# lab4d-org/lab4d

Measured on AMD Instinct MI355X. Metric: rendered rays/sec (fwd+bwd) at 512² × 128 samples; PSNR vs ref, higher is better.
Workload: dtype bf16

## Files before the change

### include/lab4d_hip.h

```cpp
#ifndef LAB4D_HIP_H
#define LAB4D_HIP_H

#include <stdint.h>

#ifdef __cplusplus
extern "C" {
#endif

#define LAB4D_OK 0
#define LAB4D_EINVAL (-1)
#define LAB4D_ELAUNCH (-2)

#define LAB4D_F32 0
#define LAB4D_F16 1
#define LAB4D_F64 2

const char* lab4d_last_error(void);
int lab4d_version(void);
const char* lab4d_arch(void);
const char* lab4d_build_flags(void);

int lab4d_quaternion_mul_forward(const void* in1, const void* in2, void* out, uint32_t B, uint32_t D1,
                                 uint32_t D2, int dtype, void* stream);
int lab4d_quaternion_mul_backward(const void* grad, uint32_t B, uint32_t D1, uint32_t D2, const void* in1,
// ... 22 lines not shown

int lab4d_sample_pdf(const float* bins, const float* weights, int R, int n_w, int n_imp, float eps,
                     float* samples, int64_t* inds, void* stream);
int lab4d_sample_pdf_u(const float* bins, const float* weights, const float* u_sorted, int R, int n_w, int n_imp, float eps,
                       float* samples, int64_t* inds, void* stream);
int lab4d_sort_depth(const float* a, int na, const float* b, int nb, int R, float* out, void* stream);

int lab4d_valid_mask(const float* xyz, const float* xyz_t, const float* aabb, const float* t_aabb, long S, unsigned char* mask, void* stream);
long lab4d_compact_work_ints(long S);
int lab4d_compact(const unsigned char* mask, long S, int* idx, int* count, int* work, void* stream);
int lab4d_gather_rows(const float* src, const int* idx, const int* count, long n_rows, int C, float* dst, void* stream);
int lab4d_scatter_rows(const float* src, const int* idx, const int* count, long n_rows, int C, float* dst, void* stream);
int lab4d_frame_of(const int* idx, const int* count, long n_rows, int spf, int* frame, void* stream);

#define LAB4D_MAX_FIELDS 16
typedef struct {
  int n_fields;
  const float* fields[LAB4D_MAX_FIELDS];
  int channels[LAB4D_MAX_FIELDS];
  int modes[LAB4D_MAX_FIELDS];
} lab4d_field_list;
typedef struct {
  int n_fields;
  float* fields[LAB4D_MAX_FIELDS];
} lab4d_field_grads;

int lab4d_composite_forward(const float* density, const float* deltas, const lab4d_field_list* fl,
                            const float* flow, const float* vis, const float* gauss_density, int R, int D,
                            float* weights, float* transmit, float* mask, float* out, float* flow_out,
                            float* vis_num, float* t_sum, float* gauss_mask, void* stream);
// ... 61 lines not shown
```

### lab4d_amd/_lib.py

```python
import ctypes
import os
import re
import subprocess
import sys
from concurrent.futures import ThreadPoolExecutor

import torch

HERE = os.path.dirname(os.path.abspath(__file__))
ROOT = os.path.dirname(HERE)
CSRC = os.path.join(HERE, "csrc")
INCLUDE = os.path.join(ROOT, "include")
SO_PATH = os.environ.get("LAB4D_SO_PATH", os.path.join(HERE, "liblab4d_hip.so"))
BUILD_DIR = os.environ.get("LAB4D_BUILD_DIR", os.path.join(HERE, "build"))
HIPCC = os.environ.get("HIPCC", "/opt/rocm/bin/hipcc")
ARCH = "gfx950"
CFLAGS = ["--offload-arch=" + ARCH, "-O3", "-std=c++17", "-fPIC", "-I" + INCLUDE, "-I" + CSRC,
          "-Wno-unused-value", "-Wno-pass-failed"] + os.environ.get("LAB4D_HIPCC_EXTRA", "").split()


MLP_INST_FLAGS = ["-mllvm", "-amdgpu-disable-unclustered-high-rp-reschedule"]


def sources():
# ... 114 lines not shown
    def bind(cls):
        MIRRORS[c_name] = cls
        if _LIB is not None:
            for name, (_, params, _) in SIGNATURES.items():
                if c_name in params:
                    getattr(_LIB, name).argtypes = argtypes(params)
        return cls
    return bind


@mirrors("lab4d_field_list")
class FieldList(ctypes.Structure):
    _fields_ = [("n_fields", ci), ("fields", vp * 16), ("channels", ci * 16), ("modes", ci * 16)]


@mirrors("lab4d_field_grads")
class FieldGrads(ctypes.Structure):
    _fields_ = [("n_fields", ci), ("fields", vp * 16)]


def lib():
    global _LIB
    if _LIB is None:
        if not os.path.exists(SO_PATH):
            raise RuntimeError(
                "liblab4d_hip.so is missing (%s). Build it with `python -c 'import __graft_entry__ as g; g.build()'`; "
                "lab4d_amd has no CPU or eager-PyTorch fallback." % SO_PATH)
        so = ctypes.CDLL(SO_PATH)
        for name, (restype, params, _) in SIGNATURES.items():
            fn = getattr(so, name)
# ... 188 lines not shown
```

### lab4d_amd/csrc/composite.hip

```cpp
#include "common.hpp"

namespace lab4d {

constexpr int kMaxChunks = 4;

template <int NC>
struct RayWeights {
  float tau[NC], w[NC], T[NC];
  float mask;
};

template <int NC>
__device__ __forceinline__ void ray_weights(const float* density, const float* deltas, long base, int D, int lane,
                                            RayWeights<NC>& rw) {
  float carry = 0.f;
  float msum = 0.f;
#pragma unroll
  for (int j = 0; j < NC; ++j) {
    const int d = lane + 64 * j;
    float tau = 0.f;
    if (d < D) tau = density[base + d] * deltas[base + d];
    const float incl = wave_scan_incl(tau, lane) + carry;
    float excl = __shfl_up(incl, 1, 64);
    if (lane == 0) excl = carry;
// ... 1 lines not shown
    const float T = expf(-incl);
    const float Tex = expf(-excl);
    const float w = (d < D) ? (1.f - expf(-tau)) * Tex : 0.f;
    rw.tau[j] = tau; rw.w[j] = w; rw.T[j] = T;
    msum += w;
  }
  rw.mask = wave_sum(msum);
}


constexpr int kMaxD = 64 * 4;
__device__ __forceinline__ int div_c(int e, int C, int sh) { return sh >= 0 ? (e >> sh) : (C == 3 ? (int)(((unsigned)e * 43691u) >> 17) : e / C); }
__device__ __forceinline__ int shift_of(int C) { return (C & (C - 1)) == 0 ? __ffs(C) - 1 : -1; }

template <int NC>
__device__ __forceinline__ void field_reduce(const float* __restrict__ v, int D, int C, const float* wl, int lane, float* __restrict__ out_c) {
  const int n = D * C, sh = shift_of(C);
  if ((64 % C) == 0) {
    float s = 0.f;
    for (int e = lane; e < n; e += 64) s += wl[e >> sh] * v[e];
    for (int o = C; o < 64; o <<= 1) s += __shfl_xor(s, o, 64);
    if (lane < C) out_c[lane] = s;
  } else if (C == 3) {
    float s0 = 0.f, s1 = 0.f, s2 = 0.f;
    for (int e = lane; e < n; e += 64) {
      const int d = div_c(e, 3, -1), c = e - 3 * d;
      const float x = wl[d] * v[e];
      s0 += c == 0 ? x : 0.f; s1 += c == 1 ? x : 0.f; s2 += c == 2 ? x : 0.f;
    }
    s0 = wave_sum(s0); s1 = wave_sum(s1); s2 = wave_sum(s2);
    if (lane == 0) { out_c[0] = s0; out_c[1] = s1; out_c[2] = s2; }
  } else {
    for (int c = 0; c < C; ++c) {
      float s = 0.f;
      for (int d = lane; d < D; d += 64) s += wl[d] * v[d * C + c];
      s = wave_sum(s);
      if (lane == 0) out_c[c] = s;
    }
  }
}

template <int NC>
__global__ void __launch_bounds__(256) k_composite_fwd(const float* __restrict__ density, const float* __restrict__ deltas,
                                                        lab4d_field_list fl, const float* __restrict__ flow,
                                                        const float* __restrict__ vis, const float* __restrict__ gdens, int R, int D,
                                                        int sumC, float* __restrict__ weights, float* __restrict__ transmit,
                                                        float* __restrict__ mask, float* __restrict__ out,
                                                        float* __restrict__ flow_out, float* __restrict__ vis_num,
                                                        float* __restrict__ t_sum, float* __restrict__ gauss_mask) {
  const int lane = threadIdx.x & 63;
  constexpr int nchunk = NC;
  __shared__ float wl_all[4][64 * NC];
  float* wl = wl_all[threadIdx.x >> 6];
  for (long ray = (long)blockIdx.x * 4 + (threadIdx.x >> 6); ray < R; ray += (long)gridDim.x * 4) {
    const long base = ray * D;
    RayWeights<NC> rw;
    ray_weights(density, deltas, base, D, lane, rw);
    const float inv = 1.f / (rw.mask + 1e-6f);
    _Pragma("unroll") for (int j = 0; j < nchunk; ++j) wl[lane + 64 * j] = rw.w[j] * inv;
    __builtin_amdgcn_wave_barrier();
    if (weights || transmit) {
      _Pragma("unroll") for (int j = 0; j < nchunk; ++j) {
        const int d = lane + 64 * j;
        if (d < D) {
          if (weights) weights[base + d] = rw.w[j];
          if (transmit) transmit[base + d] = rw.T[j];
        }
      }
    }
    if (lane == 0 && mask) mask[ray] = rw.mask;
    int co = 0;
    for (int f = 0; f < fl.n_fields; ++f) {
      const int C = fl.channels[f];
      const float* v = fl.fields[f];
      const int mode = fl.modes[f];
      const float* vr = v + base * C;
      if (mode == 2) {
        float s = 0.f;
        for (int e = lane; e < D * C; e += 64) s += vr[e];
        s = wave_sum(s);
        if (lane == 0) out[ray * sumC + co] = s / (float)(D * C);
        co += 1;
      } else {
        field_reduce<NC>(vr, D, C, wl, lane, out + ray * sumC + co);
        co += C;
      }
    }
    if (flow) {
      float sw = 0.f, su = 0.f, sv = 0.f;
      _Pragma("unroll") for (int j = 0; j < nchunk; ++j) {
        const int d = lane + 64 * j;
        if (d < D) {
          const float* f3 = flow + (base + d) * 3;
          const float wf = rw.w[j] * f3[2];
          sw += wf; su += wf * f3[0]; sv += wf * f3[1];
        }
      }
      sw = wave_sum(sw); su = wave_sum(su); sv = wave_sum(sv);
      if (lane == 0) {
// ... 6 lines not shown
      _Pragma("unroll") for (int j = 0; j < nchunk; ++j) {
        const int d = lane + 64 * j;
        if (d < D) {
          const float x = vis[base + d];
          const float ls = fminf(x, 0.f) - log1pf(expf(-fabsf(x)));
          s += ls * rw.T[j]; ts += rw.T[j];
        }
      }
      s = wave_sum(s); ts = wave_sum(ts);
      if (lane == 0) { vis_num[ray] = -s / (float)D; t_sum[ray] = ts; }
    }
    if (gdens) {
      RayWeights<NC> g;
      ray_weights(gdens, deltas, base, D, lane, g);
      if (lane == 0) gauss_mask[ray] = g.mask;
    }
  }
}

template <int NC>
__global__ void __launch_bounds__(256) k_composite_bwd(const float* __restrict__ density, const float* __restrict__ deltas,
                                                        lab4d_field_list fl, const float* __restrict__ flow,
                                                        const float* __restrict__ vis, const float* __restrict__ gdens, int R, int D,
                                                        int sumC, const float* __restrict__ g_mask, const float* __restrict__ g_out,
                                                        const float* __restrict__ g_flow_out, const float* __restrict__ g_vis_num,
                                                        const float* __restrict__ g_gauss_mask, float* __restrict__ g_density,
                                                        float* __restrict__ g_deltas, lab4d_field_grads gf,
                                                        float* __restrict__ g_flow, float* __restrict__ g_vis,
                                                        float* __restrict__ g_gdens) {
  const int lane = threadIdx.x & 63;
  constexpr int nchunk = NC;
  __shared__ float wl_all[4][64 * NC], al_all[4][64 * NC];
  float* wl = wl_all[threadIdx.x >> 6];
  float* al = al_all[threadIdx.x >> 6];
  for (long ray = (long)blockIdx.x * 4 + (threadIdx.x >> 6); ray < R; ray += (long)gridDim.x * 4) {
    const long base = ray * D;
    RayWeights<NC> rw;
    ray_weights(density, deltas, base, D, lane, rw);
    const float Z = rw.mask + 1e-6f, inv = 1.f / Z;
    float gw[NC];
    float A[NC];
#pragma unroll
    for (int j = 0; j < NC; ++j) { gw[j] = 0.f; A[j] = 0.f; wl[lane + 64 * j] = rw.w[j] * inv; al[lane + 64 * j] = 0.f; }
    __builtin_amdgcn_wave_barrier();
    int co = 0;
    for (int f = 0; f < fl.n_fields; ++f) {
      const int C = fl.channels[f];
      const float* v = fl.fields[f];
      float* gv = gf.fields[f];
      const int mode = fl.modes[f];
      const float* vr = v + base * C;
      float* gvr = gv ? gv + base * C : nullptr;
      const int n = D * C;
      if (mode == 2) {
        const float g = g_out ? g_out[ray * sumC + co] / (float)(D * C) : 0.f;
        if (gvr) for (int e = lane; e < n; e += 64) gvr[e] = g;
        co += 1;
      } else {
        const float* gc = g_out ? g_out + ray * sumC + co : nullptr;
        const int sh = shift_of(C);
        if ((64 % C) == 0) {
          const int c = lane & (C - 1);
          const float g = gc ? gc[c] : 0.f;
          for (int e = lane; e < n; e += 64) {
            const int d = e >> sh;
            if (gvr) gvr[e] = g * wl[d];
            if (mode == 0) {
              float a = g * vr[e];
              for (int o = 1; o < C; o <<= 1) a += __shfl_xor(a, o, 64);
              if (c == 0) al[d] += a;
            }
          }
        } else {
          for (int e = lane; e < n; e += 64) {
            const int d = div_c(e, C, sh), c = e - d * C;
            const float g = gc ? gc[c] : 0.f;
            if (gvr) gvr[e] = g * wl[d];
            if (mode == 0) atomicAdd(&al[d], g * vr[e]);
          }
        }
        co += C;
      }
    }
    __builtin_amdgcn_wave_barrier();
#pragma unroll
    for (int j = 0; j < NC; ++j) A[j] = al[lane + 64 * j];
    float aw = 0.f;
#pragma unroll
    for (int j = 0; j < NC; ++j) aw += A[j] * rw.w[j];
    aw = wave_sum(aw);
    const float gm = g_mask ? g_mask[ray] : 0.f;
#pragma unroll
    for (int j = 0; j < NC; ++j) gw[j] = A[j] * inv - aw * inv * inv + gm;
    if (flow) {
// ... 72 lines not shown
          const float sneg = 1.f / (1.f + expf(x));
          g_vis[base + d] = -g * rw.T[j] * sneg / (float)D;
        }
      }
    }
  }
}

}
using namespace lab4d;

static int check_fields(const lab4d_field_list* fl, int* sumC) {
  LAB4D_REQUIRE(fl && fl->n_fields >= 0 && fl->n_fields <= LAB4D_MAX_FIELDS, "composite: bad field list");
  int s = 0;
  for (int i = 0; i < fl->n_fields; ++i) {
    LAB4D_REQUIRE(fl->fields[i] && fl->channels[i] >= 1 && fl->modes[i] >= 0 && fl->modes[i] <= 2, "composite: bad field %d", i);
    s += fl->modes[i] == 2 ? 1 : fl->channels[i];
  }
  *sumC = s;
  return LAB4D_OK;
}

extern "C" int lab4d_composite_forward(const float* density, const float* deltas, const lab4d_field_list* fl, const float* flow,
                                       const float* vis, const float* gauss_density, int R, int D, float* weights,
                                       float* transmit, float* mask, float* out, float* flow_out, float* vis_num,
                                       float* t_sum, float* gauss_mask, void* stream) {
  LAB4D_REQUIRE(density && deltas, "composite_forward: null density/deltas");
  LAB4D_REQUIRE(D >= 1 && D <= 64 * kMaxChunks, "composite_forward: D must be in [1,%d] (got %d)", 64 * kMaxChunks, D);
  int sumC = 0;
  if (int e = check_fields(fl, &sumC)) return e;
  LAB4D_REQUIRE(sumC == 0 || out, "composite_forward: out is null");
  LAB4D_REQUIRE(!flow || flow_out, "composite_forward: flow_out is null");
// ... 30 lines not shown
```

### lab4d_amd/csrc/hd_math.hpp

```cpp
#pragma once
#include <math.h>
#include <stdint.h>

#if defined(__HIPCC__)
#define LAB4D_HD __host__ __device__ inline
#else
#define LAB4D_HD inline
#endif

namespace lab4d_rn {

#if defined(__HIP_DEVICE_COMPILE__)
template <typename T>
__device__ __forceinline__ void pin(T& v) { asm volatile("" : "+v"(v)); }
__device__ __forceinline__ float add_rn(float a, float b) { float p = a + b; asm volatile("" : "+v"(p)); return p; }
__device__ __forceinline__ float mul_rn(float a, float b) { float p = a * b; asm volatile("" : "+v"(p)); return p; }
__device__ __forceinline__ float div_rn(float a, float b) { return __fdiv_rn(a, b); }
__device__ __forceinline__ double dadd(double a, double b) { double p = a + b; asm volatile("" : "+v"(p)); return p; }
__device__ __forceinline__ double dmul(double a, double b) { double p = a * b; asm volatile("" : "+v"(p)); return p; }
#else
template <typename T>
LAB4D_HD void pin(T&) {}
LAB4D_HD float add_rn(float a, float b) { volatile float p = a + b; return p; }
LAB4D_HD float mul_rn(float a, float b) { volatile float p = a * b; return p; }
LAB4D_HD float div_rn(float a, float b) { volatile float p = a / b; return p; }
LAB4D_HD double dadd(double a, double b) { volatile double p = a + b; return p; }
LAB4D_HD double dmul(double a, double b) { volatile double p = a * b; return p; }
#endif

LAB4D_HD float sqrt_rn(float a) { return (float)sqrt((double)a); }
LAB4D_HD bool finite_f(float v) { return fabsf(v) <= 3.402823466e+38f; }
LAB4D_HD float inf_f() { return __builtin_huge_valf(); }
LAB4D_HD float nan_f() { return __builtin_nanf(""); }

}
```

### lab4d_amd/csrc/pointwise.hip

```cpp
#include "common.hpp"

namespace lab4d {

template <int C>
__global__ void __launch_bounds__(256) k_l2norm_fwd(const float* __restrict__ x, long S, float* __restrict__ y) {
  for (long s = (long)blockIdx.x * blockDim.x + threadIdx.x; s < S; s += (long)gridDim.x * blockDim.x) {
    float v[C];
    float q = 0.f;
#pragma unroll
    for (int c = 0; c < C; ++c) { v[c] = x[s * C + c]; q += v[c] * v[c]; }
    const float inv = 1.f / sqrtf(q);
#pragma unroll
    for (int c = 0; c < C; ++c) y[s * C + c] = v[c] * inv;
  }
}
template <int C>
__global__ void __launch_bounds__(256) k_l2norm_bwd(const float* __restrict__ x, const float* __restrict__ g, long S, float* __restrict__ gx) {
  for (long s = (long)blockIdx.x * blockDim.x + threadIdx.x; s < S; s += (long)gridDim.x * blockDim.x) {
    float v[C], gv[C];
    float q = 0.f, d = 0.f;
#pragma unroll
    for (int c = 0; c < C; ++c) { v[c] = x[s * C + c]; gv[c] = g[s * C + c]; q += v[c] * v[c]; d += v[c] * gv[c]; }
    const float inv = 1.f / sqrtf(q);
    const float k = d * inv * inv;
#pragma unroll
    for (int c = 0; c < C; ++c) gx[s * C + c] = (gv[c] - v[c] * k) * inv;
  }
}

__global__ void __launch_bounds__(256) k_eik_tangent_input(const float* __restrict__ x, const float* __restrict__ g, const float* __restrict__ ge,
                                                           const float* __restrict__ freq_w, long S, int L, int KE, float* __restrict__ u) {
  for (long s = (long)blockIdx.x * blockDim.x + threadIdx.x; s < S; s += (long)gridDim.x * blockDim.x) {
    const float g0 = g[s * 3], g1 = g[s * 3 + 1], g2 = g[s * 3 + 2];
    const float gn = sqrtf(g0 * g0 + g1 * g1 + g2 * g2);
    const float k = gn > 0.f ? ge[s] * (2.f * (gn - 1.f) / fmaxf(gn, 1e-38f)) : 0.f;
    const float d[3] = {k * g0, k * g1, k * g2};
    const float xv[3] = {x[s * 3], x[s * 3 + 1], x[s * 3 + 2]};
    float* row = u + s * KE;
    for (int f = 0; f < L; ++f) {
      const float fr = ldexpf(1.f, f);
      const float wf = freq_w ? fr * freq_w[f] : fr;
// ... 43 lines not shown
```

### lab4d_amd/deformable.py

```python
import ctypes
import os

import torch
import torch.nn.functional as F
from torch.autograd import Function
from torch.autograd.function import once_differentiable

from . import _lib, mlp
from . import quat_utils as Q
from . import render_utils as RU
from .warping import composed_warp, dense_warp, skinning_warp, skinning_warp_forward_multi

vp, ci, cf = ctypes.c_void_p, ctypes.c_int, ctypes.c_float


def flip_pair(x):
    if torch.is_tensor(x):
        if len(x) < 2:
            return x
        return x.view(x.shape[0] // 2, 2, -1).flip(1).view(x.shape)
    if isinstance(x, tuple):
        return tuple(flip_pair(t) for t in x)
    if isinstance(x, dict):
        return {k: flip_pair(v) for k, v in x.items()}
# ... 122 lines not shown

def volsdf_density(sdf, logibeta):
    return VolSdfDensity.apply(sdf, logibeta.exp())


EIK_REUSE = os.environ.get("LAB4D_EIK_REUSE", "1") != "0"


def posenc_window(alpha, n_freq, device):
    if alpha is None:
        return None
    w = torch.clamp(alpha * n_freq - torch.arange(n_freq, dtype=torch.float32, device=device), 0.0, 1.0)
    return 0.5 * (1 + torch.cos(torch.pi * w + torch.pi))


def nerf_forward(P, xyz, fr, prec, with_color=True, get_density=True, alpha=None, ft=None, tap=None):
    shape = xyz.shape
    spf = _spf(xyz)
    x = xyz.reshape(-1, 3)
    dev = x.device
    r = mlp.run_chain(mlp.NET_FG_BASE, prec, P, x, spf, conds={0: fr["code_base"], 4: fr["code_base"]}, export_layer=8 if with_color else None,
                      freq_w=posenc_window(alpha, 10, dev), pfs_pre=None if ft is None else {0: ft["pf.base0"], 4: ft["pf.base4"]}, tap=tap)
    sdf, feat = r if with_color else (r, None)
    sdf = sdf.view(shape[:-1] + (1,))
    if get_density:
        out = volsdf_density(sdf, P["logibeta"])
    else:
        out = sdf
    if not with_color:
        return out
    rgb = mlp.run_chain(mlp.NET_FG_COLOR, prec, P, x, spf, conds={0: fr["code_color"], 3: fr["appr_code"]}, ext=feat,
                        freq_w=posenc_window(alpha, 12, dev), pfs_pre=None if ft is None else {0: ft["pf.color0"], 3: ft["pf.color3"]})
    return torch.sigmoid(rgb).view(shape[:-1] + (3,)), out


def nerf_forward_bg(P, xyz, dir, codes, prec, get_density=True, alpha=None, prefix="", tap=None):
    shape = xyz.shape
    spf = _spf(xyz)
    x = xyz.reshape(-1, 3)
    dev = x.device
    r = mlp.run_chain(mlp.NET_BG_BASE, prec, P, x, spf, conds={0: codes["basefield"], 4: codes["basefield"]}, export_layer=5 if dir is not None else None,
                      freq_w=posenc_window(alpha, 6, dev), prefix=prefix, tap=tap)
    sdf, feat = r if dir is not None else (r, None)
    sdf = sdf.view(shape[:-1] + (1,))
    if get_density:
        out = volsdf_density(sdf, P[prefix + "logibeta"])
    else:
        out = sdf
# ... 20 lines not shown
        y = torch.empty_like(x)
        _lib.call("l2_normalize_forward", x, S, C, y)
        ctx.save_for_backward(x)
        return y

    @staticmethod
    @once_differentiable
    def backward(ctx, g):
        (x,) = ctx.saved_tensors
        g = g.contiguous()
        gx = torch.empty_like(x)
        _lib.call("l2_normalize_backward", x, g, x.shape[0], x.shape[1], gx)
        return gx


def compute_feat(P, xyz, prec):
    f = mlp.run_chain(mlp.NET_FEAT, prec, P, xyz.reshape(-1, 3), _spf(xyz))
    return L2Normalize.apply(f).view(xyz.shape[:-1] + (16,))


class GlobalMatch(Function):

    @staticmethod
    def forward(ctx, feat_px, feat_c, xyz_c, logsigma):
        feat_px, feat_c, xyz_c, logsigma = [t.detach().contiguous().float() for t in (feat_px, feat_c, xyz_c, logsigma)]
        _lib.require_device(feat_px, feat_c, xyz_c, logsigma)
        R, C = feat_px.shape
        K = feat_c.shape[0]
        out = torch.empty(R, 3, device=feat_px.device)
        stats = torch.empty(R, 2, device=feat_px.device)
        with _lib.timed("k_match_fwd", (2.0 * R * K * (C + 3), 4.0 * (R * (C + 5) + K * (C + 3)))):
            _lib.call("global_match_forward", feat_px, feat_c, xyz_c, logsigma, R, C, K, out, stats)
        ctx.save_for_backward(feat_px, feat_c, xyz_c, logsigma, out, stats)
# ... 180 lines not shown

    def warp(x, t_art, rest_art, t_embed, backward, partner=False):
        if motion == "rigid":
            return x, {}
        if motion == "dense":
            te = flip_pair(fr["t_embed_dense"]) if partner else fr["t_embed_dense"]
            return dense_warp(P, x, te, fr["code_dense_bw" if backward else "code_dense_fw"], backward, prec, prefix="warp.", net=mlp.NET_DENSE6), {}
        if dense is None:
            return skinning_warp(P, x, t_art, rest_art, t_embed, fr["code_skin"], backward, prec)
        d = dict(dense, t_embed=flip_pair(dense["t_embed"])) if partner else dense
        return composed_warp(P, x, t_art, rest_art, t_embed, fr["code_skin"], backward, prec, dense=d)

    return warp


def query_field_train(P, fr, hxy, rng, flow_thresh=None, n_depth=64, alpha=None, prec=mlp.PREC_F32):
    warp = _warp_fn(P, fr, prec)
    ft = fr.get("frame_terms")
    if ft is None:
        ft = frame_terms(P, fr)
    motion = fr.get("motion", "skinning")
    skinning = fr.get("dense") is None and motion == "skinning"
    cam2field = (ft["cam2field.q"], ft["cam2field.t"])
    xyz_cam, dir_cam, deltas, depth, xyz_t, _ = RU.ray_samples(hxy, fr["Kinv"], fr["near_far"], cam2field, n_depth=n_depth)
    t_art, rest_art = fr.get("t_articulation"), fr.get("rest_articulation")
    if skinning:
        xyz, bw_aux = skinning_warp(P, xyz_t, t_art, rest_art, fr["t_embed"], fr["code_skin"], True, prec,
                                    pre={"se3": (ft["se3_bw.r"], ft["se3_bw.d"]), "gauss": ft["gauss"], "pf": ft["pf.skin_bw"], "tab": ft.get("skinA.bw")})
    else:
        xyz, bw_aux = warp(xyz_t, t_art, rest_art, fr.get("t_embed"), True)
    matching = fr.get("feature") is not None
    if matching:
        xyz_flat, xyz_rows = RowTap.apply(xyz.reshape(-1, 3), rng["match_perm"])
        xyz = xyz_flat.view(xyz.shape)
    fd = {}
    vis = vis_field(P, xyz, fr, prec, ft)
    base_tap = {} if EIK_REUSE else None
    rgb, density = nerf_forward(P, xyz, fr, prec, alpha=alpha, ft=ft, tap=base_tap)
    fd["rgb"], fd["density"], fd["density_fg"], fd["vis"] = rgb, density, density, vis
    nxt = flip_pair({k: fr.get(k) for k in ["Kinv", "field2cam", "t_articulation", "rest_articulation"]})
    shared = skinning and fr.get("rest_shared_in_pair", True)
    fw_pre = {"gauss": ft["gauss"], "pf": ft["pf.skin_fw"], "tab": ft.get("skinA.fw")} if skinning else None
    if shared:
        (xyz_next, _), (xyz_cyc, cyc_aux) = skinning_warp_forward_multi(P, xyz, [nxt["t_articulation"], t_art], rest_art,
                                                                        fr["t_embed_mean"], fr["code_skin"], prec,
                                                                        pre=dict(fw_pre, se3s=[(ft["se3_next.r"], ft["se3_next.d"]), (ft["se3_own.r"], ft["se3_own.d"])]))
    else:
        xyz_next, _ = warp(xyz, nxt["t_articulation"], nxt["rest_articulation"], fr.get("t_embed_mean"), False, partner=True)
    if not shared:
        xyz_cyc, cyc_aux = warp(xyz, t_art, rest_art, fr.get("t_embed_mean"), False)
    fd["flow"], fd["cyc_dist"] = FlowCyc.apply(xyz_next, ft["field2cam_next.q"], ft["field2cam_next.t"], ft["Kmat_next"], hxy, xyz_cyc, xyz_t, flow_thresh)
    for k in ["skin_entropy", "delta_skin"]:
        fd[k] = (cyc_aux[k] + bw_aux[k]) / 2 if k in cyc_aux else torch.zeros_like(fd["cyc_dist"])
    fd["eikonal"] = eikonal_subsample(P, xyz, fr["code_base"], rng.get("eik_inds"), alpha, prec, pf_tables=(ft["pf.base0"], ft["pf.base4"]), tap=base_tap)
    fd["xyz"] = xyz
    fd["xyz_cam"] = xyz_cam
    fd["depth"] = depth / ft["scale"]
    fd["feature"] = compute_feat(P, xyz, prec)
    aux = {}
    has_gauss = motion not in ("rigid", "dense")
    if not matching:
        if has_gauss:
            fd["gauss_density"] = gauss_density(P, xyz, rest_art, ft)
        return fd, deltas, aux
    feat_flat, feat_rows = RowTap.apply(fd["feature"].reshape(-1, fd["feature"].shape[-1]), rng["match_perm"])
    fd["feature"] = feat_flat.view(fd["feature"].shape)
    xyz_matches = global_match(P, fr["feature"], feat_rows, xyz_rows)
    if skinning:
        xm_next, _ = skinning_warp(P, xyz_matches[:, :, None], t_art, rest_art, fr["t_embed_mean"], fr["code_skin"], False,
                                   prec, pre=dict(fw_pre, se3=(ft["se3_own.r"], ft["se3_own.d"])))
    else:
        xm_next, _ = warp(xyz_matches[:, :, None], t_art, rest_art, fr.get("t_embed_mean"), False)
    xyz_reproj = rigid_apply(fr["field2cam"][0], fr["field2cam"][1], xm_next)[:, :, 0]
    aux["xyz_matches"] = xyz_matches
    aux["xyz_reproj"] = xyz_reproj
    aux["xy_reproj"] = pinhole_projection(ft["Kmat"], xyz_reproj)[..., :2]
    if has_gauss:
        fd["gauss_density"] = gauss_density(P, xyz, rest_art, ft)
    return fd, deltas, aux


def render_train(P, fr, hxy, rng, flow_thresh=None, n_depth=64, alpha=None, prec=mlp.PREC_F32):
    fd, deltas, aux = query_field_train(P, fr, hxy, rng, flow_thresh, n_depth, alpha, prec)
    rendered = RU.render_pixel(fd, deltas)
    aux_fg = dict(aux)
    aux_fg.update(rendered)
    rendered = dict(rendered)
    rendered["xyz_matches"] = aux["xyz_matches"]
    rendered["xyz_reproj"] = aux["xyz_reproj"]
    return {"rendered": rendered, "aux_dict": {"fg": aux_fg}}


def mask_balance_wt(mask, vis2d, is_detected):
    mask = mask.float()
    vis2d = vis2d.float() * is_detected.float()[:, None, None]
    vis = (vis2d > 0).float()
    npos, nneg = (mask * vis).sum(), ((1 - mask) * vis).sum()
    pos = vis2d.sum() / npos.clamp_min(1e-12)
    neg = vis2d.sum() / nneg.clamp_min(1e-12)
# ... 382 lines not shown
```

### lab4d_amd/render_utils.py

```python
import torch
import torch.nn.functional as F
from torch.autograd import Function
from torch.autograd.function import once_differentiable

from . import _lib

KEY_SKIP = ["density", "vis", "flow", "eikonal", "xy_reproj", "xyz_reproj", "gauss_density"]
KEY_FREEZE = ["cyc_dist", "xyz_cam", "skin_entropy"]
KEY_MEAN = ["eikonal", "delta_skin"]


def _f32(*ts):
    _lib.require_device(*ts)
    for t in ts:
        if t is not None and t.dtype != torch.float32:
            raise RuntimeError("this op is fp32 only (the reference path is fp32, SURVEY F6); got %s" % t.dtype)


class _RaySamples(Function):

    @staticmethod
    def forward(ctx, hxy, Kinv, near_far, depth_in, cq, ct, D):
        hxy, Kinv = hxy.contiguous(), Kinv.contiguous()
        near_far = near_far.contiguous() if near_far is not None else None
# ... 44 lines not shown
            z = torch.linspace(0, 1, n_depth, device=hxy.device)[None]
            depth = (near_far[:, 0:1] * (1 - z) + near_far[:, 1:2] * z)[:, None, :, None].repeat(1, N, 1, 1)
        mid = 0.5 * (depth[:, :, :-1] + depth[:, :, 1:])
        upper = torch.cat([mid, depth[:, :, -1:]], -2)
        lower = torch.cat([depth[:, :, :1], mid], -2)
        depth = (lower + (upper - lower) * torch.rand(depth.shape, device=hxy.device)).contiguous()
    return _RaySamples.apply(hxy, Kinv, near_far, depth, None, None, n_depth)[:4]


def ray_samples(hxy, Kinv, near_far, cam2field, n_depth=64, depth=None):
    return _RaySamples.apply(hxy, Kinv, near_far, depth, cam2field[0], cam2field[1], n_depth)


class _Composite(Function):
    @staticmethod
    def forward(ctx, density, deltas, flow, vis, gdens, modes, *fields):
        M, N, D = density.shape[:3]
        R = M * N
        density, deltas = density.contiguous(), deltas.contiguous()
        fields = [f.contiguous() for f in fields]
        flow = flow.contiguous() if flow is not None else None
        vis = vis.contiguous() if vis is not None else None
        gdens = gdens.contiguous() if gdens is not None else None
        _f32(density, deltas, flow, vis, gdens, *fields)
        dev = density.device
        fl = _lib.FieldList()
        fl.n_fields = len(fields)
        sumC = 0
        for i, (f, m) in enumerate(zip(fields, modes)):
            fl.fields[i] = _lib.dp(f)
            fl.channels[i] = f.shape[-1]
            fl.modes[i] = m
            sumC += 1 if m == 2 else f.shape[-1]
        weights = torch.empty(M, N, D, device=dev)
        transmit = torch.empty(M, N, D, device=dev)
        mask = torch.empty(M, N, 1, device=dev)
        out = torch.empty(M, N, max(sumC, 1), device=dev)
        flow_out = torch.empty(M, N, 2, device=dev) if flow is not None else None
        vis_num = torch.empty(M, N, 1, device=dev) if vis is not None else None
        t_sum = torch.empty(M, N, 1, device=dev) if vis is not None else None
        gmask = torch.empty(M, N, 1, device=dev) if gdens is not None else None
        extra = (3 if flow is not None else 0) + (1 if vis is not None else 0) + (1 if gdens is not None else 0)
        chans = sum(f.shape[-1] for f in fields)
        ctx.chans = chans + extra
        with _lib.timed("k_composite_fwd", (0.0, 4.0 * R * D * (2 + chans + extra + 2))):
            _lib.call("composite_forward", density, deltas, fl, flow, vis, gdens, R, D, weights, transmit, mask, out, flow_out, vis_num, t_sum, gmask)
        ctx.save_for_backward(density, deltas, flow, vis, gdens, *fields)
        ctx.modes = tuple(modes)
        ctx.dims = (M, N, D, sumC)
        ctx.mark_non_differentiable(weights, transmit)
        if t_sum is not None:
            ctx.mark_non_differentiable(t_sum)
        return mask, out, flow_out, vis_num, t_sum, gmask, weights, transmit

    @staticmethod
    @once_differentiable
    def backward(ctx, g_mask, g_out, g_flow_out, g_vis_num, g_t_sum, g_gmask, g_w, g_T):
        density, deltas, flow, vis, gdens, *fields = ctx.saved_tensors
        M, N, D, sumC = ctx.dims
        R = M * N

        def c(g):
            return g.contiguous() if g is not None else None

        g_mask, g_out, g_flow_out, g_vis_num, g_gmask = c(g_mask), c(g_out), c(g_flow_out), c(g_vis_num), c(g_gmask)
        fl = _lib.FieldList()
        gf = _lib.FieldGrads()
        fl.n_fields = gf.n_fields = len(fields)
        gfields = []
        for i, (f, m) in enumerate(zip(fields, ctx.modes)):
            fl.fields[i] = _lib.dp(f)
            fl.channels[i] = f.shape[-1]
            fl.modes[i] = m
            need = ctx.needs_input_grad[6 + i]
            g = torch.empty_like(f) if need else None
            gfields.append(g)
            gf.fields[i] = _lib.dp(g) if g is not None else None
        g_density = torch.empty_like(density)
        g_deltas = torch.empty_like(deltas)
        g_flow = torch.empty_like(flow) if (flow is not None and ctx.needs_input_grad[2]) else None
        g_vis = torch.empty_like(vis) if (vis is not None and ctx.needs_input_grad[3]) else None
        g_gd = torch.empty_like(gdens) if (gdens is not None and ctx.needs_input_grad[4]) else None
        with _lib.timed("k_composite_bwd", (0.0, 4.0 * R * D * 2 * (2 + ctx.chans))):
            _lib.call("composite_backward", density, deltas, fl, flow, vis, gdens, R, D, g_mask, g_out, g_flow_out, g_vis_num, g_gmask, g_density, g_deltas, gf,
                      g_flow, g_vis, g_gd)
        return (g_density, g_deltas, g_flow, g_vis, g_gd, None, *gfields)


def _composite(field_dict, deltas):
    keys, modes, fields = [], [], []
    for k, v in field_dict.items():
        if k in KEY_MEAN:
            keys.append(k); modes.append(2); fields.append(v)
        elif k in KEY_SKIP:
            continue
        else:
            keys.append(k); modes.append(1 if k in KEY_FREEZE else 0); fields.append(v)
    flow = field_dict.get("flow")
    vis = field_dict.get("vis")
    gd = field_dict.get("gauss_density")
    if len(fields) > 16:
        raise RuntimeError("render_pixel: more than 16 fields")
    res = _Composite.apply(field_dict["density"], deltas, flow, vis, gd, tuple(modes), *fields)
    return keys, modes, fields, res


class _Weights(Function):

    @staticmethod
    def forward(ctx, density, deltas):
        res = _Composite.apply(density.detach(), deltas.detach(), None, None, None, ())
        w, T = res[6], res[7]
        ctx.save_for_backward(density, deltas, w, T)
        ctx.mark_non_differentiable(T)
        return w, T

    @staticmethod
    @once_differentiable
    def backward(ctx, gw, gT):
        density, deltas, w, T = ctx.saved_tensors
        x = gw * w
        suffix = torch.flip(torch.cumsum(torch.flip(x, [-1]), -1), [-1]) - x
        gtau = (gw * T - suffix)[..., None]
        return gtau * deltas, gtau * density


# ... 15 lines not shown
        wf = weights * field_dict["flow"][..., 2]
        wf = wf / (wf.sum(-1, keepdim=True) + 1e-6)
        out["flow"] = (wf.unsqueeze(-1) * field_dict["flow"][..., :2]).sum(-2)
    if "normal" in field_dict:
        out["normal"] = F.normalize(out["normal"], 2, -1)
    dkeys = [k for k in out if "density_" in k]
    if dkeys:
        dsum = torch.cat([out[k] for k in dkeys], -1).sum(-1, keepdim=True) + 1e-6
        for k in dkeys:
            out[k.replace("density_", "mask_")] = out[k] / dsum
            del out[k]
    return out


def render_pixel(field_dict, deltas):
    keys, modes, fields, (mask, out, flow_out, vis_num, t_sum, gmask, w, T) = _composite(field_dict, deltas)
    rendered = {"mask": mask}
    co = 0
    for k, m, f in zip(keys, modes, fields):
        c = 1 if m == 2 else f.shape[-1]
        v = out[..., co:co + c]
        co += c
        rendered[k] = v[..., 0] if m == 2 else v
    if flow_out is not None:
        rendered["flow"] = flow_out
    if "normal" in rendered:
        rendered["normal"] = F.normalize(rendered["normal"], 2, -1)
    dkeys = [k for k in rendered if "density_" in k]
    if dkeys:
        dsum = torch.cat([rendered[k] for k in dkeys], -1).sum(-1, keepdim=True) + 1e-6
        for k in dkeys:
# ... 137 lines not shown
```

Baseline: 746,300.

## Fuse sigmoid and L2-normalize activations into the composite kernels

Passes raw RGB logits and raw feature vectors into the compositing kernels, tagged with an activation code packed into the field mode, and applies sigmoid or per-sample L2 normalization inside the forward and backward reductions. This removes the separate elementwise activation kernels and their full-size intermediate tensors over every sample. In exchange the composite kernels recompute the activation in backward, and the L2 path adds a per-ray inverse-norm pass into shared memory. The matching branch still normalizes the gathered feature rows separately.

```diff
diff --git a/include/lab4d_hip.h b/include/lab4d_hip.h
--- a/include/lab4d_hip.h
+++ b/include/lab4d_hip.h
@@ -60,6 +60,11 @@
 int lab4d_frame_of(const int* idx, const int* count, long n_rows, int spf, int* frame, void* stream);
 
 #define LAB4D_MAX_FIELDS 16
+#define LAB4D_ACT_NONE 0
+#define LAB4D_ACT_SIGMOID 1
+#define LAB4D_ACT_L2NORM 2
+#define LAB4D_FIELD_MODE(m) ((m) & 0xff)
+#define LAB4D_FIELD_ACT(m) ((int)((unsigned)(m) >> 8))
 typedef struct {
   int n_fields;
   const float* fields[LAB4D_MAX_FIELDS];
diff --git a/lab4d_amd/_lib.py b/lab4d_amd/_lib.py
--- a/lab4d_amd/_lib.py
+++ b/lab4d_amd/_lib.py
@@ -152,6 +152,9 @@
     _fields_ = [("n_fields", ci), ("fields", vp * 16), ("channels", ci * 16), ("modes", ci * 16)]
 
 
+ACT_NONE, ACT_SIGMOID, ACT_L2NORM = 0, 1, 2
+
+
 @mirrors("lab4d_field_grads")
 class FieldGrads(ctypes.Structure):
     _fields_ = [("n_fields", ci), ("fields", vp * 16)]
diff --git a/lab4d_amd/csrc/composite.hip b/lab4d_amd/csrc/composite.hip
--- a/lab4d_amd/csrc/composite.hip
+++ b/lab4d_amd/csrc/composite.hip
@@ -39,18 +39,44 @@
 __device__ __forceinline__ int shift_of(int C) { return (C & (C - 1)) == 0 ? __ffs(C) - 1 : -1; }
 
 template <int NC>
-__device__ __forceinline__ void field_reduce(const float* __restrict__ v, int D, int C, const float* wl, int lane, float* __restrict__ out_c) {
+__device__ __forceinline__ void sample_inv_norms(const float* __restrict__ vr, int D, int lane, float* il) {
+#pragma unroll 1
+  for (int j = 0; j < NC; ++j) {
+    const int d = lane + 64 * j;
+    if (d < D) {
+      const float4* p = reinterpret_cast<const float4*>(vr + d * 16);
+      float q = 0.f;
+#pragma unroll 1
+      for (int k = 0; k < 4; ++k) {
+        const float4 a = p[k];
+        const float x[4] = {a.x, a.y, a.z, a.w};
+        q = lab4d_act::l2norm_sq(x, 4, q);
+      }
+      il[d] = lab4d_act::l2norm_inv(q);
+    }
+  }
+  __builtin_amdgcn_wave_barrier();
+}
+template <int ACT>
+__device__ __forceinline__ float act_of(float x, const float* il, int d) {
+  if (ACT == LAB4D_ACT_SIGMOID) return lab4d_act::sigmoid(x);
+  if (ACT == LAB4D_ACT_L2NORM) return x * il[d];
+  return x;
+}
+
+template <int NC, int ACT>
+__device__ __forceinline__ void field_reduce(const float* __restrict__ v, int D, int C, const float* wl, const float* il, int lane, float* __restrict__ out_c) {
   const int n = D * C, sh = shift_of(C);
   if ((64 % C) == 0) {
     float s = 0.f;
-    for (int e = lane; e < n; e += 64) s += wl[e >> sh] * v[e];
+    for (int e = lane; e < n; e += 64) s += wl[e >> sh] * act_of<ACT>(v[e], il, e >> sh);
     for (int o = C; o < 64; o <<= 1) s += __shfl_xor(s, o, 64);
     if (lane < C) out_c[lane] = s;
   } else if (C == 3) {
     float s0 = 0.f, s1 = 0.f, s2 = 0.f;
     for (int e = lane; e < n; e += 64) {
       const int d = div_c(e, 3, -1), c = e - 3 * d;
-      const float x = wl[d] * v[e];
+      const float x = wl[d] * act_of<ACT>(v[e], il, d);
       s0 += c == 0 ? x : 0.f; s1 += c == 1 ? x : 0.f; s2 += c == 2 ? x : 0.f;
     }
     s0 = wave_sum(s0); s1 = wave_sum(s1); s2 = wave_sum(s2);
@@ -58,7 +84,7 @@
   } else {
     for (int c = 0; c < C; ++c) {
       float s = 0.f;
-      for (int d = lane; d < D; d += 64) s += wl[d] * v[d * C + c];
+      for (int d = lane; d < D; d += 64) s += wl[d] * act_of<ACT>(v[d * C + c], il, d);
       s = wave_sum(s);
       if (lane == 0) out_c[c] = s;
     }
@@ -75,8 +101,9 @@
                                                         float* __restrict__ t_sum, float* __restrict__ gauss_mask) {
   const int lane = threadIdx.x & 63;
   constexpr int nchunk = NC;
-  __shared__ float wl_all[4][64 * NC];
+  __shared__ float wl_all[4][64 * NC], il_all[4][64 * NC];
   float* wl = wl_all[threadIdx.x >> 6];
+  float* il = il_all[threadIdx.x >> 6];
   for (long ray = (long)blockIdx.x * 4 + (threadIdx.x >> 6); ray < R; ray += (long)gridDim.x * 4) {
     const long base = ray * D;
     RayWeights<NC> rw;
@@ -98,7 +125,7 @@
     for (int f = 0; f < fl.n_fields; ++f) {
       const int C = fl.channels[f];
       const float* v = fl.fields[f];
-      const int mode = fl.modes[f];
+      const int mode = LAB4D_FIELD_MODE(fl.modes[f]);
       const float* vr = v + base * C;
       if (mode == 2) {
         float s = 0.f;
@@ -107,7 +134,16 @@
         if (lane == 0) out[ray * sumC + co] = s / (float)(D * C);
         co += 1;
       } else {
-        field_reduce<NC>(vr, D, C, wl, lane, out + ray * sumC + co);
+        float* oc = out + ray * sumC + co;
+        const int act = LAB4D_FIELD_ACT(fl.modes[f]);
+        if (act == LAB4D_ACT_L2NORM) {
+          sample_inv_norms<NC>(vr, D, lane, il);
+          field_reduce<NC, LAB4D_ACT_L2NORM>(vr, D, C, wl, il, lane, oc);
+        } else if (act == LAB4D_ACT_SIGMOID) {
+          field_reduce<NC, LAB4D_ACT_SIGMOID>(vr, D, C, wl, il, lane, oc);
+        } else {
+          field_reduce<NC, LAB4D_ACT_NONE>(vr, D, C, wl, il, lane, oc);
+        }
         co += C;
       }
     }
@@ -144,6 +180,58 @@
       RayWeights<NC> g;
       ray_weights(gdens, deltas, base, D, lane, g);
       if (lane == 0) gauss_mask[ray] = g.mask;
+    }
+  }
+}
+
+template <int ACT>
+__device__ __forceinline__ void field_adjoint(const float* __restrict__ vr, float* __restrict__ gvr, const float* __restrict__ gc, int n, int C, int mode,
+                                              const float* wl, const float* il, float* al, int lane) {
+  const int sh = shift_of(C);
+  if ((64 % C) == 0) {
+    const int c = lane & (C - 1);
+    const float g = gc ? gc[c] : 0.f;
+    for (int e = lane; e < n; e += 64) {
+      const int d = e >> sh;
+      if (ACT == LAB4D_ACT_NONE) {
+        if (gvr) gvr[e] = g * wl[d];
+        if (mode == 0) {
+          float a = g * vr[e];
+          for (int o = 1; o < C; o <<= 1) a += __shfl_xor(a, o, 64);
+          if (c == 0) al[d] += a;
+        }
+      } else {
+        const float x = vr[e], gy = g * wl[d];
+        float y;
+        if (ACT == LAB4D_ACT_SIGMOID) {
+          y = lab4d_act::sigmoid(x);
+          if (gvr) gvr[e] = lab4d_act::sigmoid_bwd(gy, y);
+        } else {
+          const float inv = il[d];
+          y = x * inv;
+          float dot = x * gy;
+          for (int o = 1; o < C; o <<= 1) dot += __shfl_xor(dot, o, 64);
+          if (gvr) gvr[e] = lab4d_act::l2norm_bwd(gy, x, lab4d_act::l2norm_bwd_k(dot, inv), inv);
+        }
+        if (mode == 0) {
+          float a = g * y;
+          for (int o = 1; o < C; o <<= 1) a += __shfl_xor(a, o, 64);
+          if (c == 0) al[d] += a;
+        }
+      }
+    }
+  } else {
+    for (int e = lane; e < n; e += 64) {
+      const int d = div_c(e, C, sh), c = e - d * C;
+      const float g = gc ? gc[c] : 0.f;
+      if (ACT == LAB4D_ACT_NONE) {
+        if (gvr) gvr[e] = g * wl[d];
+        if (mode == 0) atomicAdd(&al[d], g * vr[e]);
+      } else {
+        const float y = lab4d_act::sigmoid(vr[e]);
+        if (gvr) gvr[e] = lab4d_act::sigmoid_bwd(g * wl[d], y);
+        if (mode == 0) atomicAdd(&al[d], g * y);
+      }
     }
   }
 }
@@ -160,8 +248,9 @@
                                                         float* __restrict__ g_gdens) {
   const int lane = threadIdx.x & 63;
   constexpr int nchunk = NC;
-  __shared__ float wl_all[4][64 * NC], al_all[4][64 * NC];
+  __shared__ float wl_all[4][64 * NC], al_all[4][64 * NC], il_all[4][64 * NC];
   float* wl = wl_all[threadIdx.x >> 6];
+  float* il = il_all[threadIdx.x >> 6];
   float* al = al_all[threadIdx.x >> 6];
   for (long ray = (long)blockIdx.x * 4 + (threadIdx.x >> 6); ray < R; ray += (long)gridDim.x * 4) {
     const long base = ray * D;
@@ -178,7 +267,7 @@
       const int C = fl.channels[f];
       const float* v = fl.fields[f];
       float* gv = gf.fields[f];
-      const int mode = fl.modes[f];
+      const int mode = LAB4D_FIELD_MODE(fl.modes[f]);
       const float* vr = v + base * C;
       float* gvr = gv ? gv + base * C : nullptr;
       const int n = D * C;
@@ -188,26 +277,14 @@
         co += 1;
       } else {
         const float* gc = g_out ? g_out + ray * sumC + co : nullptr;
-        const int sh = shift_of(C);
-        if ((64 % C) == 0) {
-          const int c = lane & (C - 1);
-          const float g = gc ? gc[c] : 0.f;
-          for (int e = lane; e < n; e += 64) {
-            const int d = e >> sh;
-            if (gvr) gvr[e] = g * wl[d];
-            if (mode == 0) {
-              float a = g * vr[e];
-              for (int o = 1; o < C; o <<= 1) a += __shfl_xor(a, o, 64);
-              if (c == 0) al[d] += a;
-            }
-          }
+        const int act = LAB4D_FIELD_ACT(fl.modes[f]);
+        if (act == LAB4D_ACT_L2NORM) {
+          sample_inv_norms<NC>(vr, D, lane, il);
+          field_adjoint<LAB4D_ACT_L2NORM>(vr, gvr, gc, n, C, mode, wl, il, al, lane);
+        } else if (act == LAB4D_ACT_SIGMOID) {
+          field_adjoint<LAB4D_ACT_SIGMOID>(vr, gvr, gc, n, C, mode, wl, il, al, lane);
         } else {
-          for (int e = lane; e < n; e += 64) {
-            const int d = div_c(e, C, sh), c = e - d * C;
-            const float g = gc ? gc[c] : 0.f;
-            if (gvr) gvr[e] = g * wl[d];
-            if (mode == 0) atomicAdd(&al[d], g * vr[e]);
-          }
+          field_adjoint<LAB4D_ACT_NONE>(vr, gvr, gc, n, C, mode, wl, il, al, lane);
         }
         co += C;
       }
@@ -310,8 +387,13 @@
   LAB4D_REQUIRE(fl && fl->n_fields >= 0 && fl->n_fields <= LAB4D_MAX_FIELDS, "composite: bad field list");
   int s = 0;
   for (int i = 0; i < fl->n_fields; ++i) {
-    LAB4D_REQUIRE(fl->fields[i] && fl->channels[i] >= 1 && fl->modes[i] >= 0 && fl->modes[i] <= 2, "composite: bad field %d", i);
-    s += fl->modes[i] == 2 ? 1 : fl->channels[i];
+    const int mode = LAB4D_FIELD_MODE(fl->modes[i]), act = LAB4D_FIELD_ACT(fl->modes[i]);
+    LAB4D_REQUIRE(fl->fields[i] && fl->channels[i] >= 1 && fl->modes[i] >= 0 && mode <= 2, "composite: bad field %d", i);
+    LAB4D_REQUIRE(act == LAB4D_ACT_NONE || act == LAB4D_ACT_SIGMOID || act == LAB4D_ACT_L2NORM, "composite: field %d has the unknown activation %d", i, act);
+    LAB4D_REQUIRE(act == LAB4D_ACT_NONE || mode != 2, "composite: field %d is a plain mean (mode 2) and takes no activation", i);
+    LAB4D_REQUIRE(act != LAB4D_ACT_L2NORM || (fl->channels[i] == 16 && ((uintptr_t)fl->fields[i] & 15) == 0),
+                  "composite: an L2NORM field has 16 channels and a 16-byte aligned base (field %d: %d channels)", i, fl->channels[i]);
+    s += mode == 2 ? 1 : fl->channels[i];
   }
   *sumC = s;
   return LAB4D_OK;
diff --git a/lab4d_amd/csrc/hd_math.hpp b/lab4d_amd/csrc/hd_math.hpp
--- a/lab4d_amd/csrc/hd_math.hpp
+++ b/lab4d_amd/csrc/hd_math.hpp
@@ -34,3 +34,23 @@
 LAB4D_HD float nan_f() { return __builtin_nanf(""); }
 
 }
+
+namespace lab4d_act {
+
+LAB4D_HD float l2norm_sq(const float* x, int C, float q = 0.f) {
+  for (int c = 0; c < C; ++c) q = lab4d_rn::add_rn(q, lab4d_rn::mul_rn(x[c], x[c]));
+  return q;
+}
+LAB4D_HD float l2norm_inv(float q) { return 1.f / sqrtf(q); }
+LAB4D_HD float l2norm_dot(const float* x, const float* g, int C) {
+  float d = 0.f;
+  for (int c = 0; c < C; ++c) d = lab4d_rn::add_rn(d, lab4d_rn::mul_rn(x[c], g[c]));
+  return d;
+}
+LAB4D_HD float l2norm_bwd_k(float dot, float inv) { return dot * inv * inv; }
+LAB4D_HD float l2norm_bwd(float g, float x, float k, float inv) { return fmaf(-x, k, g) * inv; }
+
+LAB4D_HD float sigmoid(float x) { return 1.f / (1.f + expf(-x)); }
+LAB4D_HD float sigmoid_bwd(float g, float y) { return g * y * (1.f - y); }
+
+}
diff --git a/lab4d_amd/csrc/pointwise.hip b/lab4d_amd/csrc/pointwise.hip
--- a/lab4d_amd/csrc/pointwise.hip
+++ b/lab4d_amd/csrc/pointwise.hip
@@ -6,10 +6,9 @@
 __global__ void __launch_bounds__(256) k_l2norm_fwd(const float* __restrict__ x, long S, float* __restrict__ y) {
   for (long s = (long)blockIdx.x * blockDim.x + threadIdx.x; s < S; s += (long)gridDim.x * blockDim.x) {
     float v[C];
-    float q = 0.f;
 #pragma unroll
-    for (int c = 0; c < C; ++c) { v[c] = x[s * C + c]; q += v[c] * v[c]; }
-    const float inv = 1.f / sqrtf(q);
+    for (int c = 0; c < C; ++c) v[c] = x[s * C + c];
+    const float inv = lab4d_act::l2norm_inv(lab4d_act::l2norm_sq(v, C));
 #pragma unroll
     for (int c = 0; c < C; ++c) y[s * C + c] = v[c] * inv;
   }
@@ -18,13 +17,12 @@
 __global__ void __launch_bounds__(256) k_l2norm_bwd(const float* __restrict__ x, const float* __restrict__ g, long S, float* __restrict__ gx) {
   for (long s = (long)blockIdx.x * blockDim.x + threadIdx.x; s < S; s += (long)gridDim.x * blockDim.x) {
     float v[C], gv[C];
-    float q = 0.f, d = 0.f;
 #pragma unroll
-    for (int c = 0; c < C; ++c) { v[c] = x[s * C + c]; gv[c] = g[s * C + c]; q += v[c] * v[c]; d += v[c] * gv[c]; }
-    const float inv = 1.f / sqrtf(q);
-    const float k = d * inv * inv;
+    for (int c = 0; c < C; ++c) { v[c] = x[s * C + c]; gv[c] = g[s * C + c]; }
+    const float inv = lab4d_act::l2norm_inv(lab4d_act::l2norm_sq(v, C));
+    const float k = lab4d_act::l2norm_bwd_k(lab4d_act::l2norm_dot(v, gv, C), inv);
 #pragma unroll
-    for (int c = 0; c < C; ++c) gx[s * C + c] = (gv[c] - v[c] * k) * inv;
+    for (int c = 0; c < C; ++c) gx[s * C + c] = lab4d_act::l2norm_bwd(gv[c], v[c], k, inv);
   }
 }
 
diff --git a/lab4d_amd/deformable.py b/lab4d_amd/deformable.py
--- a/lab4d_amd/deformable.py
+++ b/lab4d_amd/deformable.py
@@ -160,7 +160,7 @@
     return 0.5 * (1 + torch.cos(torch.pi * w + torch.pi))
 
 
-def nerf_forward(P, xyz, fr, prec, with_color=True, get_density=True, alpha=None, ft=None, tap=None):
+def nerf_forward(P, xyz, fr, prec, with_color=True, get_density=True, alpha=None, ft=None, tap=None, raw_rgb=False):
     shape = xyz.shape
     spf = _spf(xyz)
     x = xyz.reshape(-1, 3)
@@ -177,7 +177,7 @@
         return out
     rgb = mlp.run_chain(mlp.NET_FG_COLOR, prec, P, x, spf, conds={0: fr["code_color"], 3: fr["appr_code"]}, ext=feat,
                         freq_w=posenc_window(alpha, 12, dev), pfs_pre=None if ft is None else {0: ft["pf.color0"], 3: ft["pf.color3"]})
-    return torch.sigmoid(rgb).view(shape[:-1] + (3,)), out
+    return (rgb if raw_rgb else torch.sigmoid(rgb)).view(shape[:-1] + (3,)), out
 
 
 def nerf_forward_bg(P, xyz, dir, codes, prec, get_density=True, alpha=None, prefix="", tap=None):
@@ -228,9 +228,9 @@
         return gx
 
 
-def compute_feat(P, xyz, prec):
+def compute_feat(P, xyz, prec, raw=False):
     f = mlp.run_chain(mlp.NET_FEAT, prec, P, xyz.reshape(-1, 3), _spf(xyz))
-    return L2Normalize.apply(f).view(xyz.shape[:-1] + (16,))
+    return (f if raw else L2Normalize.apply(f)).view(xyz.shape[:-1] + (16,))
 
 
 class GlobalMatch(Function):
@@ -441,7 +441,7 @@
     return warp
 
 
-def query_field_train(P, fr, hxy, rng, flow_thresh=None, n_depth=64, alpha=None, prec=mlp.PREC_F32):
+def query_field_train(P, fr, hxy, rng, flow_thresh=None, n_depth=64, alpha=None, prec=mlp.PREC_F32, fuse_acts=False):
     warp = _warp_fn(P, fr, prec)
     ft = fr.get("frame_terms")
     if ft is None:
@@ -463,8 +463,10 @@
     fd = {}
     vis = vis_field(P, xyz, fr, prec, ft)
     base_tap = {} if EIK_REUSE else None
-    rgb, density = nerf_forward(P, xyz, fr, prec, alpha=alpha, ft=ft, tap=base_tap)
+    rgb, density = nerf_forward(P, xyz, fr, prec, alpha=alpha, ft=ft, tap=base_tap, raw_rgb=fuse_acts)
     fd["rgb"], fd["density"], fd["density_fg"], fd["vis"] = rgb, density, density, vis
+    acts = {"rgb": "sigmoid", "feature": "l2norm"} if fuse_acts else None
+    ret = (lambda *r: r + (acts,)) if fuse_acts else (lambda *r: r)
     nxt = flip_pair({k: fr.get(k) for k in ["Kinv", "field2cam", "t_articulation", "rest_articulation"]})
     shared = skinning and fr.get("rest_shared_in_pair", True)
     fw_pre = {"gauss": ft["gauss"], "pf": ft["pf.skin_fw"], "tab": ft.get("skinA.fw")} if skinning else None
@@ -483,15 +485,17 @@
     fd["xyz"] = xyz
     fd["xyz_cam"] = xyz_cam
     fd["depth"] = depth / ft["scale"]
-    fd["feature"] = compute_feat(P, xyz, prec)
+    fd["feature"] = compute_feat(P, xyz, prec, raw=fuse_acts)
     aux = {}
     has_gauss = motion not in ("rigid", "dense")
     if not matching:
         if has_gauss:
             fd["gauss_density"] = gauss_density(P, xyz, rest_art, ft)
-        return fd, deltas, aux
+        return ret(fd, deltas, aux)
     feat_flat, feat_rows = RowTap.apply(fd["feature"].reshape(-1, fd["feature"].shape[-1]), rng["match_perm"])
     fd["feature"] = feat_flat.view(fd["feature"].shape)
+    if fuse_acts:
+        feat_rows = L2Normalize.apply(feat_rows)
     xyz_matches = global_match(P, fr["feature"], feat_rows, xyz_rows)
     if skinning:
         xm_next, _ = skinning_warp(P, xyz_matches[:, :, None], t_art, rest_art, fr["t_embed_mean"], fr["code_skin"], False,
@@ -504,12 +508,12 @@
     aux["xy_reproj"] = pinhole_projection(ft["Kmat"], xyz_reproj)[..., :2]
     if has_gauss:
         fd["gauss_density"] = gauss_density(P, xyz, rest_art, ft)
-    return fd, deltas, aux
+    return ret(fd, deltas, aux)
 
 
 def render_train(P, fr, hxy, rng, flow_thresh=None, n_depth=64, alpha=None, prec=mlp.PREC_F32):
-    fd, deltas, aux = query_field_train(P, fr, hxy, rng, flow_thresh, n_depth, alpha, prec)
-    rendered = RU.render_pixel(fd, deltas)
+    fd, deltas, aux, acts = query_field_train(P, fr, hxy, rng, flow_thresh, n_depth, alpha, prec, fuse_acts=True)
+    rendered = RU.render_pixel_tagged(fd, deltas, acts)
     aux_fg = dict(aux)
     aux_fg.update(rendered)
     rendered = dict(rendered)
diff --git a/lab4d_amd/render_utils.py b/lab4d_amd/render_utils.py
--- a/lab4d_amd/render_utils.py
+++ b/lab4d_amd/render_utils.py
@@ -82,7 +82,7 @@
 
 class _Composite(Function):
     @staticmethod
-    def forward(ctx, density, deltas, flow, vis, gdens, modes, *fields):
+    def forward(ctx, density, deltas, flow, vis, gdens, modes, acts, *fields):
         M, N, D = density.shape[:3]
         R = M * N
         density, deltas = density.contiguous(), deltas.contiguous()
@@ -95,10 +95,11 @@
         fl = _lib.FieldList()
         fl.n_fields = len(fields)
         sumC = 0
-        for i, (f, m) in enumerate(zip(fields, modes)):
+        acts = tuple(acts) if acts else (_lib.ACT_NONE,) * len(fields)
+        for i, (f, m, a) in enumerate(zip(fields, modes, acts)):
             fl.fields[i] = _lib.dp(f)
             fl.channels[i] = f.shape[-1]
-            fl.modes[i] = m
+            fl.modes[i] = m | (a << 8)
             sumC += 1 if m == 2 else f.shape[-1]
         weights = torch.empty(M, N, D, device=dev)
         transmit = torch.empty(M, N, D, device=dev)
@@ -114,7 +115,7 @@
         with _lib.timed("k_composite_fwd", (0.0, 4.0 * R * D * (2 + chans + extra + 2))):
             _lib.call("composite_forward", density, deltas, fl, flow, vis, gdens, R, D, weights, transmit, mask, out, flow_out, vis_num, t_sum, gmask)
         ctx.save_for_backward(density, deltas, flow, vis, gdens, *fields)
-        ctx.modes = tuple(modes)
+        ctx.modes, ctx.acts = tuple(modes), acts
         ctx.dims = (M, N, D, sumC)
         ctx.mark_non_differentiable(weights, transmit)
         if t_sum is not None:
@@ -136,11 +137,11 @@
         gf = _lib.FieldGrads()
         fl.n_fields = gf.n_fields = len(fields)
         gfields = []
-        for i, (f, m) in enumerate(zip(fields, ctx.modes)):
+        for i, (f, m, a) in enumerate(zip(fields, ctx.modes, ctx.acts)):
             fl.fields[i] = _lib.dp(f)
             fl.channels[i] = f.shape[-1]
-            fl.modes[i] = m
-            need = ctx.needs_input_grad[6 + i]
+            fl.modes[i] = m | (a << 8)
+            need = ctx.needs_input_grad[7 + i]
             g = torch.empty_like(f) if need else None
             gfields.append(g)
             gf.fields[i] = _lib.dp(g) if g is not None else None
@@ -152,10 +153,13 @@
         with _lib.timed("k_composite_bwd", (0.0, 4.0 * R * D * 2 * (2 + ctx.chans))):
             _lib.call("composite_backward", density, deltas, fl, flow, vis, gdens, R, D, g_mask, g_out, g_flow_out, g_vis_num, g_gmask, g_density, g_deltas, gf,
                       g_flow, g_vis, g_gd)
-        return (g_density, g_deltas, g_flow, g_vis, g_gd, None, *gfields)
-
-
-def _composite(field_dict, deltas):
+        return (g_density, g_deltas, g_flow, g_vis, g_gd, None, None, *gfields)
+
+
+ACTS = {"sigmoid": _lib.ACT_SIGMOID, "l2norm": _lib.ACT_L2NORM}
+
+
+def _composite(field_dict, deltas, acts=None):
     keys, modes, fields = [], [], []
     for k, v in field_dict.items():
         if k in KEY_MEAN:
@@ -164,12 +168,16 @@
             continue
         else:
             keys.append(k); modes.append(1 if k in KEY_FREEZE else 0); fields.append(v)
+    unknown = set(acts or ()) - set(keys)
+    if unknown:
+        raise KeyError("render_pixel: activation tags for %s, which are not composited fields" % sorted(unknown))
+    tags = tuple(ACTS[acts[k]] if acts and k in acts else _lib.ACT_NONE for k in keys)
     flow = field_dict.get("flow")
     vis = field_dict.get("vis")
     gd = field_dict.get("gauss_density")
     if len(fields) > 16:
         raise RuntimeError("render_pixel: more than 16 fields")
-    res = _Composite.apply(field_dict["density"], deltas, flow, vis, gd, tuple(modes), *fields)
+    res = _Composite.apply(field_dict["density"], deltas, flow, vis, gd, tuple(modes), tags, *fields)
     return keys, modes, fields, res
 
 
@@ -177,7 +185,7 @@
 
     @staticmethod
     def forward(ctx, density, deltas):
-        res = _Composite.apply(density.detach(), deltas.detach(), None, None, None, ())
+        res = _Composite.apply(density.detach(), deltas.detach(), None, None, None, (), ())
         w, T = res[6], res[7]
         ctx.save_for_backward(density, deltas, w, T)
         ctx.mark_non_differentiable(T)
@@ -223,7 +231,11 @@
 
 
 def render_pixel(field_dict, deltas):
-    keys, modes, fields, (mask, out, flow_out, vis_num, t_sum, gmask, w, T) = _composite(field_dict, deltas)
+    return render_pixel_tagged(field_dict, deltas, None)
+
+
+def render_pixel_tagged(field_dict, deltas, acts):
+    keys, modes, fields, (mask, out, flow_out, vis_num, t_sum, gmask, w, T) = _composite(field_dict, deltas, acts)
     rendered = {"mask": mask}
     co = 0
     for k, m, f in zip(keys, modes, fields):
```

Result: no change. 750,200, median of 6 (+0.5%).
